# tum-pbs/differentiable-piso

Hardware: AMD Instinct MI355X
Metric: PISO steps/s (fwd+adjoint) at 2048^2 staggered grid (higher is better)
Workload: dtype f64

## Files before the change

### differentiable-piso_amd/csrc/cg.hip

```cpp
#include <atomic>
#include "cg_kernels.h"
#include "cg_driver.h"
#include "cg_tiny.h"
#include "options.h"
#include <cstdio>
#include <vector>

namespace piso {

struct CgProfile {
  int enabled = 0, stride = 8;
  double ms[4] = {0, 0, 0, 0};
  long long count[4] = {0, 0, 0, 0};
};
static CgProfile g_prof;

struct HostPoll {
  CgState* pinned = nullptr;
  hipEvent_t ev[2] = {nullptr, nullptr};
  hipEvent_t seg_ev[2] = {nullptr, nullptr};
  int cus = 0;
};
static std::atomic<unsigned> g_persist_launches{0};
static int g_persist_fallbacks = 0;
static thread_local int tl_xcd_map[kPersistMaxGrid];
static thread_local int tl_xcd_map_n = 0;
static long long g_tiny_solves = 0;
enum { DI_PATH = 0, DI_SIZEOF_T, DI_SIZEOF_CT, DI_V, DI_RECON, DI_SYMMETRIC, DI_ROWS_PER_WAVE, DI_K1_GRID, DI_K1_TILES, DI_R, DI_NQ,
       DI_WAVES, DI_LAUNCH_GRID, DI_PADDED, DI_XCD_LOCAL, DI_FELL_BACK, DI_TINY_PER_X, DI_K2_GRID, DI_SEGMENTS, DI_COUNT };
static thread_local int tl_dispatch[DI_COUNT];
static thread_local int tl_dispatch_n = 0;
static bool g_xcd_local_failed = false;
static long long g_verify_runs = 0;
static int g_verify_failures = 0;
constexpr int kPollDevices = 16;
static thread_local HostPoll tl_poll_dev[kPollDevices];
static thread_local HostPoll* tl_poll_cur = &tl_poll_dev[0];
#define tl_poll (*tl_poll_cur)

static int ensure_poll() {
  int dev = 0;
  PISO_HIP_CHECK(hipGetDevice(&dev));
  if (dev < 0 || dev >= kPollDevices) { set_error_msg("piso_cg_solve: device ordinal out of range"); return PISO_ERR_INVALID_ARG; }
  tl_poll_cur = &tl_poll_dev[dev];
  if (!tl_poll.pinned) {
    PISO_HIP_CHECK(hipHostMalloc(reinterpret_cast<void**>(&tl_poll.pinned), 2 * sizeof(CgState), hipHostMallocDefault));
    PISO_HIP_CHECK(hipEventCreateWithFlags(&tl_poll.ev[0], hipEventDisableTiming));
    PISO_HIP_CHECK(hipEventCreateWithFlags(&tl_poll.ev[1], hipEventDisableTiming));
    PISO_HIP_CHECK(hipDeviceGetAttribute(&tl_poll.cus, hipDeviceAttributeMultiprocessorCount, dev));
  }
  return PISO_OK;
}

constexpr size_t kPadMaxCells = (size_t)1 << 19;
static bool padded_dims(int nx, int ny, int per_x, int per_y, int elem, int* nxp, int* nyp) {
  *nxp = nx; *nyp = ny;
  if (elem != 8 || nx % 2 != 0 || nx < 8 || ny < 8) return false;
  const bool pad_x = nx % 128 != 0, pad_y = ny % 2 != 0;
  if (!pad_x && !pad_y) return false;
  const int px = (nx + 127) / 128 * 128;
  int py = (ny + 3) / 4 * 4;
  if (px != nx && per_x) return false;
  if (py != ny && per_y) {
    py = ny;
    if (ny % 2 != 0 || ((long long)(px / 128) * (ny / 2)) % 2 != 0) return false;
  }
  if ((size_t)px * py > kPadMaxCells) return false;
  *nxp = px; *nyp = py;
  return true;
}

template <typename T>
struct CgCarve { T *cC, *oT; float* oF; int* flags; T *b_pad, *x_pad; unsigned* persist_ws; };
template <typename T>
static CgCarve<T> cg_carve(Arena& ar, size_t n, bool padded, CgArgs<T>& a) {
  CgCarve<T> c;
  c.cC = ar.take<T>(n);
  c.oT = ar.take<T>(4 * n);
  c.oF = ar.take<float>(4 * n);
  c.flags = ar.take<int>(4);
  c.b_pad = padded ? ar.take<T>(n) : nullptr;
  c.x_pad = padded ? ar.take<T>(n) : nullptr;
  a.r = ar.take<T>(n); a.z = ar.take<T>(n); a.p[0] = ar.take<T>(n); a.p[1] = ar.take<T>(n);
  a.zp[0] = ar.take<T>(n); a.zp[1] = ar.take<T>(n);
  a.partsA = ar.take<T>(3 * kMaxPartials); a.partsB = ar.take<T>(3 * kMaxPartials); a.partsS = ar.take<T>(kMaxPartials);
  a.scal = ar.take<T>(SC_COUNT);
  a.state = ar.take<CgState>(2);
  c.persist_ws = ar.take<unsigned>(kPersistWsWordsAll);
  return c;
}

template <typename T>
static size_t cg_workspace_bytes(int nx_in, int ny_in) {
  int nx = nx_in, ny = ny_in;
  const bool padded = padded_dims(nx_in, ny_in, 0, 0, (int)sizeof(T), &nx, &ny);
  Arena ar = counting_arena();
  CgArgs<T> a;
  cg_carve<T>(ar, (padded ? 3 : 1) * (size_t)nx * ny, false, a);
  return counted_bytes(ar);
}

static void record_dispatch(int path, size_t state_bytes, size_t coef_bytes, int tiny_per_x, int V = 0, bool recon = false, bool symmetric = false,
                            const CgTiling* t = nullptr, const PersistPlan* p = nullptr, bool fell_back = false) {
  int* d = tl_dispatch;
  for (int i = 0; i < DI_COUNT; ++i) d[i] = 0;
  d[DI_PATH] = path; d[DI_SIZEOF_T] = (int)state_bytes; d[DI_SIZEOF_CT] = (int)coef_bytes; d[DI_TINY_PER_X] = tiny_per_x;
  d[DI_V] = V; d[DI_RECON] = recon ? 1 : 0; d[DI_SYMMETRIC] = symmetric ? 1 : 0; d[DI_FELL_BACK] = fell_back ? 1 : 0;
  if (t) { d[DI_ROWS_PER_WAVE] = t->rows_per_wave; d[DI_K1_GRID] = t->g1; d[DI_K1_TILES] = t->k1_tiles; d[DI_K2_GRID] = t->g2; }
  if (p) d[DI_PADDED] = p->ragged ? 1 : 0;
  if (p && p->R) { d[DI_R] = p->R; d[DI_NQ] = p->NQ; d[DI_WAVES] = p->waves; d[DI_LAUNCH_GRID] = p->launch_grid; d[DI_XCD_LOCAL] = p->xcd_local ? 1 : 0; }
  tl_dispatch_n = DI_COUNT;
}

struct EventPool {
  static constexpr int kMax = 64;
  hipEvent_t start[2][kMax], stop[2][kMax];
  int used[2] = {0, 0};
  bool created = false;
};
static thread_local EventPool tl_events;
struct SegmentTimes { double ms = 0; long long iters = 0, launches = 0; };

static int ensure_events(EventPool& ep) {
  if (ep.created) return PISO_OK;
  for (int q = 0; q < 2; ++q)
    for (int i = 0; i < EventPool::kMax; ++i) {
      PISO_HIP_CHECK(hipEventCreate(&ep.start[q][i]));
      PISO_HIP_CHECK(hipEventCreate(&ep.stop[q][i]));
    }
  ep.created = true;
  return PISO_OK;
}

static int read_profile(const EventPool& ep, const SegmentTimes& seg, float* kernel_ms_out) {
  double ms[2] = {0, 0};
  for (int q = 0; q < 2; ++q)
    for (int i = 0; i < ep.used[q]; ++i) {
      float t = 0;
      PISO_HIP_CHECK(hipEventElapsedTime(&t, ep.start[q][i], ep.stop[q][i]));
      ms[q] += t;
    }
  if (kernel_ms_out) {
    kernel_ms_out[0] = ep.used[0] ? (float)(ms[0] / ep.used[0]) : 0.f;
    kernel_ms_out[1] = ep.used[1] ? (float)(ms[1] / ep.used[1]) : 0.f;
  }
  if (g_prof.enabled) {
    for (int q = 0; q < 2; ++q) { g_prof.ms[q] += ms[q]; g_prof.count[q] += ep.used[q]; }
    g_prof.ms[2] += seg.ms; g_prof.count[2] += seg.iters; g_prof.count[3] += seg.launches;
  }
  if (kernel_ms_out && seg.iters > 0) { kernel_ms_out[0] = (float)(seg.ms / seg.iters); kernel_ms_out[1] = 0.f; }
  return PISO_OK;
}

struct PersistTiming {
  unsigned long long* ticks = nullptr;
  ~PersistTiming() { if (ticks) (void)hipFree(ticks); }
};
static int print_persist_timing(const unsigned long long* ticks, int grid, int k_last) {
  std::vector<unsigned long long> h(12 * grid);
  PISO_HIP_CHECK(hipMemcpy(h.data(), ticks, h.size() * sizeof(unsigned long long), hipMemcpyDeviceToHost));
  const char* names[9] = {"D (p update, stencil, sums, publish)", "exchange", "U (stencil, x / r update, ring)", "-", "-",
                           "  exchange: wave sums + drain of the perimeter stores", "  exchange: first barrier", "  exchange: publish + polling",
                           "  exchange: record sums + second barrier"};
  const double f = 0.01 / (double)(k_last > 0 ? k_last : 1);
  if (opt(OPT_CG_PERSIST_TIMING) >= 2) {
    for (int b = 0; b < grid; ++b)
      fprintf(stderr, "cg_persist_wg %3d xcd %d band %3d  D %.2f  exchange %.2f  U %.2f  | drain %.2f  barrier1 %.2f  publish+poll %.2f  sums %.2f\n", b, (int)h[9 * grid + b], (int)h[10 * grid + b],
              f * (double)h[0 * grid + b], f * (double)h[1 * grid + b], f * (double)h[2 * grid + b],
              f * (double)h[5 * grid + b], f * (double)h[6 * grid + b], f * (double)h[7 * grid + b], f * (double)h[8 * grid + b]);
  }
  for (int q = 0; q < 9; ++q) {
    double s = 0, mn = 1e300, mx = 0;
    for (int b = 0; b < grid; ++b) { const double v = (double)h[q * grid + b]; s += v; mn = v < mn ? v : mn; mx = v > mx ? v : mx; }
    fprintf(stderr, "cg_persist %s: avg %.2f us/iter  min %.2f  max %.2f\n", names[q], f * s / grid, f * mn, f * mx);
  }
  return PISO_OK;
}

template <typename T, typename CT>
static int verify_residual(const CgArgs<T>& a, const PersistCtl& pc, hipStream_t stream, bool* failed) {
  unsigned* out2 = reinterpret_cast<unsigned*>(pc.err) + 4;
  PISO_HIP_CHECK(hipMemsetAsync(out2, 0, 2 * sizeof(unsigned), stream));
  const int gvf = grid_for((long long)a.nx * a.ny, kBlock * 4, 1024);
  cg_verify_sum_x<T><<<gvf, kBlock, 0, stream>>>(a, a.partsA);
  cg_verify_gap<T, CT><<<gvf, kBlock, 0, stream>>>(a, a.partsA, gvf, out2);
  PISO_LAUNCH_CHECK();
  unsigned h2[2] = {0, 0};
  PISO_HIP_CHECK(hipMemcpyAsync(h2, out2, sizeof(h2), hipMemcpyDeviceToHost, stream));
  PISO_HIP_CHECK(hipStreamSynchronize(stream));
  float gap, scale;
  memcpy(&gap, &h2[0], 4); memcpy(&scale, &h2[1], 4);
  ++g_verify_runs;
  *failed = (gap > 1e-5f * scale && gap > 1e-30f) || opt(OPT_CG_VERIFY) == 2;
  return PISO_OK;
}

static int inspect_poll(int slot, int* stop_it) {
  hipError_t e = hipEventSynchronize(tl_poll.ev[slot]);
  if (e != hipSuccess) { set_error("hipEventSynchronize", e); return -1; }
  if (tl_poll.pinned[slot].done) { *stop_it = tl_poll.pinned[slot].iterations; return 1; }
  return 0;
}
static int poll_batch(size_t n) {
  const double t_iter_us = (double)n * 120.0 / 4.0e6;
  const int batch = (int)(1000.0 / (t_iter_us < 8.0 ? 8.0 : t_iter_us));
  return batch < 10 ? 10 : (batch > 200 ? 200 : batch);
}

template <typename T, typename CT, int V, bool RECON>
struct GpuLink {
  CgArgs<T> a;
  hipStream_t stream;
  bool fixed, prof;
  CgTiling tile;
  PersistPlan plan;
  PersistCtl pc;
  PersistTiming timing;
  int seg_len, batch, prof_stride, polls = 0, unsynced = 0;
  bool sample = false;
  SegmentTimes seg;
  EventPool& ep = tl_events;

  int start(unsigned* persist_ws, bool symmetric, int rank_deficient, bool allow_persist) {
    const size_t n = (size_t)a.nx * a.ny;
    tile = cg_tile(a, V, opt(OPT_CG_RPW), opt(OPT_CG_MAXBLOCKS));
    PISO_TRY(ensure_poll());
    if (prof) PISO_TRY(ensure_events(ep));
    ep.used[0] = ep.used[1] = 0;
    prof_stride = g_prof.stride > 0 ? g_prof.stride : 8;
    cg_init<T><<<tile.gflat, kBlock, 0, stream>>>(a, rank_deficient);
    PISO_LAUNCH_CHECK();
    batch = poll_batch(n);
    plan = persist_plan(PersistQuery{a.nx, a.ny, V, a.per_y, a.nx_true != 0, sizeof(T), sizeof(CT), RECON, symmetric, false, tl_poll.cus,
                                     opt(OPT_CG_PERSIST), opt(OPT_CG_PERSIST_R), opt(OPT_CG_PERSIST_HALF), opt(OPT_CG_PERSIST_NQ),
                                     opt(OPT_CG_XCD_LOCAL), g_xcd_local_failed, allow_persist});
    PISO_TRY((persist_prepare<T, CT, RECON, false>(plan, tl_poll.cus, pc, persist_ws, stream)));
    if (plan.R && kPersistDiag && opt_on(OPT_CG_PERSIST_TIMING)) {
      PISO_HIP_CHECK(hipMalloc(reinterpret_cast<void**>(&timing.ticks), 12 * plan.launch_grid * sizeof(unsigned long long)));
      PISO_HIP_CHECK(hipMemsetAsync(timing.ticks, 0, 12 * plan.launch_grid * sizeof(unsigned long long), stream));
      pc.timing = timing.ticks;
    }
    record_dispatch(plan.R ? 3 : 2, sizeof(T), sizeof(CT), 0, V, RECON, symmetric, &tile, &plan, !allow_persist);
    seg_len = persist_segment_len(n, opt(OPT_CG_SEGMENT));
    hipEvent_t* seg_ev = tl_poll.seg_ev;
    if (plan.R && prof && !seg_ev[0]) { PISO_HIP_CHECK(hipEventCreate(&seg_ev[0])); PISO_HIP_CHECK(hipEventCreate(&seg_ev[1])); }
    return PISO_OK;
  }

  bool persistent() const { return plan.R != 0; }
  int segment(int k, int ke, CgLoop& st) {
    hipEvent_t* seg_ev = tl_poll.seg_ev;
    if (prof) PISO_HIP_CHECK(hipEventRecord(seg_ev[0], stream));
    PISO_TRY((persist_launch<T, CT, RECON, false>(plan, a, pc, g_persist_launches.fetch_add(1, std::memory_order_relaxed), k, ke, st.sv, st.pending, NoSlab{}, stream)));
    if (prof) PISO_HIP_CHECK(hipEventRecord(seg_ev[1], stream));
    const bool defer = !prof && ke - k <= 32 && unsynced + (ke - k) <= 256 && ke < st.total;
    unsynced = defer ? unsynced + (ke - k) : 0;
    if (defer) return PISO_OK;
    PISO_HIP_CHECK(hipMemcpyAsync(&tl_poll.pinned[0], &a.state[0], sizeof(CgState), hipMemcpyDeviceToHost, stream));
    int herr = 0;
    PISO_HIP_CHECK(hipMemcpyAsync(&herr, pc.err, sizeof(int), hipMemcpyDeviceToHost, stream));
    PISO_HIP_CHECK(hipStreamSynchronize(stream));
    if (herr) {
      ++g_persist_fallbacks;
      if (plan.xcd_local) g_xcd_local_failed = true;
      return kPersistRetry;
    }
    const CgState& hst = tl_poll.pinned[0];
    if (prof) {
      const int ran = hst.done ? (hst.iterations - k > 0 ? hst.iterations - k : 0) : ke - k;
      float t = 0; PISO_HIP_CHECK(hipEventElapsedTime(&t, seg_ev[0], seg_ev[1])); seg.ms += t; seg.iters += ran < ke - k ? ran : ke - k; ++seg.launches;
    }
    if (hst.done) { st.finished = true; st.stop_it = hst.iterations; }
    return PISO_OK;
  }

  int k1(int k, int mode, int sv, int chk, int pend) {
    sample = prof && mode == MODE_NORMAL && (k % prof_stride == prof_stride - 1) && ep.used[0] < EventPool::kMax;
    if (sample) PISO_HIP_CHECK(hipEventRecord(ep.start[0][ep.used[0]], stream));
    cg_k1<T, CT, V, RECON><<<tile.g1, kBlock, 0, stream>>>(a, k, mode, sv, chk, pend);
    if (sample) PISO_HIP_CHECK(hipEventRecord(ep.stop[0][ep.used[0]++], stream));
    return PISO_OK;
  }
  int k2(int k, int sv) {
    if (sample) PISO_HIP_CHECK(hipEventRecord(ep.start[1][ep.used[1]], stream));
    cg_k2<T, V><<<tile.g2, kBlock, 0, stream>>>(a, k, sv);
    if (sample) PISO_HIP_CHECK(hipEventRecord(ep.stop[1][ep.used[1]++], stream));
    return PISO_OK;
  }
  int flush(int k, int sv) { cg_flush_x<T><<<tile.gflat, kBlock, 0, stream>>>(a, k, sv); return PISO_OK; }
  int reset_residual(int sv) { cg_reset_residual<T><<<tile.gflat, kBlock, 0, stream>>>(a, sv); return PISO_OK; }
  int halo(int) { return PISO_OK; }

  int poll(CgLoop& st, bool now) {
    const int slot = polls & 1;
    PISO_HIP_CHECK(hipMemcpyAsync(&tl_poll.pinned[slot], &a.state[st.sv & 1], sizeof(CgState), hipMemcpyDeviceToHost, stream));
    PISO_HIP_CHECK(hipEventRecord(tl_poll.ev[slot], stream));
    if (now || polls > 0) {
      const int r = inspect_poll(now ? slot : (polls - 1) & 1, &st.stop_it);
      if (r < 0) return PISO_ERR_HIP;
      if (r > 0) st.finished = true;
    }
    ++polls;
    return PISO_OK;
  }
  int look(int k, CgLoop& st) { return (!fixed && (k + 1) % batch == 0 && k + 1 < st.total) ? poll(st, false) : PISO_OK; }

  int finish(CgLoop& st) {
    if (!fixed && !st.finished) PISO_TRY(poll(st, true));
    PISO_HIP_CHECK(hipStreamSynchronize(stream));
    if (opt(OPT_CG_XCD_MAP) == 1) {
      tl_xcd_map_n = 0;
      if (st.segments_run > 0 && !plan.xcd_local && plan.grid <= kPersistMaxGrid) {
        PISO_HIP_CHECK(hipMemcpy(tl_xcd_map, pc.xcd + kPersistXcdTable, (size_t)plan.grid * sizeof(int), hipMemcpyDeviceToHost));
        tl_xcd_map_n = plan.grid;
      }
    }
    if (st.segments_run > 0) {
      int herr = 0;
      PISO_HIP_CHECK(hipMemcpy(&herr, pc.err, sizeof(int), hipMemcpyDeviceToHost));
      if (herr) { ++g_persist_fallbacks; return kPersistRetry; }
    }
    if (st.segments_run > 0 && sizeof(T) == 8 && !fixed && opt(OPT_CG_VERIFY) != 0) {
      bool failed = false;
      PISO_TRY((verify_residual<T, CT>(a, pc, stream, &failed)));
      if (failed) { ++g_verify_failures; ++g_persist_fallbacks; return kPersistRetry; }
    }
    if (timing.ticks) PISO_TRY(print_persist_timing(timing.ticks, plan.grid, st.k_last));
    tl_dispatch[DI_SEGMENTS] = st.segments_run;
    return PISO_OK;
  }
};

template <typename T>
__global__ __launch_bounds__(kBlock) void cg_copy_rows(const T* __restrict__ src, T* __restrict__ dst, int nx, int ny, int ld_src, int ld_dst) {
  const size_t n = (size_t)nx * ny;
  for (size_t i = (size_t)blockIdx.x * kBlock + threadIdx.x; i < n; i += (size_t)gridDim.x * kBlock) {
    const size_t j = i / (size_t)nx, c = i % (size_t)nx;
    dst[j * (size_t)ld_dst + c] = src[j * (size_t)ld_src + c];
  }
}

template <typename T>
static int cg_solve(int nx, int ny, int per_x, int per_y, const T* L, const T* b, T* x_out, float accuracy,
                    int max_iterations, int rank_deficient, int reset, int fixed, int* iterations_out,
                    float* kernel_ms_out, void* ws, size_t ws_bytes, piso_stream_t stream_, int* iterations_dev = nullptr) {
  tl_dispatch_n = 0;
  if (nx < 1 || ny < 1 || !L || !b || !x_out || !ws || max_iterations < 0 || reset < 1) {
    set_error_msg("piso_cg_solve: invalid argument");
    return PISO_ERR_INVALID_ARG;
  }
  if (ws_bytes < cg_workspace_bytes<T>(nx, ny)) {
    set_error_msg("piso_cg_solve: workspace too small");
    return PISO_ERR_INVALID_ARG;
  }
  hipStream_t stream = static_cast<hipStream_t>(stream_);
  const size_t n_true = (size_t)nx * ny;
  if (n_true <= (size_t)kTinyMaxCells && opt(OPT_CG_TINY) != 0 && opt(OPT_CG_PERSIST) < 0) {
    CgState* st_dev = reinterpret_cast<CgState*>(ws);
    const int total = fixed ? fixed : max_iterations;
    hipEvent_t* ev = nullptr;
    if (kernel_ms_out) {
      { const int rc = ensure_poll(); if (rc != PISO_OK) return rc; }
      ev = tl_poll.seg_ev;
      if (!ev[0]) { PISO_HIP_CHECK(hipEventCreate(&ev[0])); PISO_HIP_CHECK(hipEventCreate(&ev[1])); }
      PISO_HIP_CHECK(hipEventRecord(ev[0], stream));
    }
    const bool async = iterations_dev != nullptr;
    const bool cols = nx <= 64 && ny <= kColsMaxNy && (!per_x || nx == 64) && opt(OPT_CG_TINY) != 2;
    if (cols && per_x)
      cg_tiny_cols<T, true><<<1, kTinyThreads, 0, stream>>>(L, b, x_out, nx, ny, per_y, fixed ? -1.0f : accuracy, total, fixed ? 0 : reset,
                                                            rank_deficient, st_dev, iterations_dev);
    else if (cols)
      cg_tiny_cols<T, false><<<1, kTinyThreads, 0, stream>>>(L, b, x_out, nx, ny, per_y, fixed ? -1.0f : accuracy, total, fixed ? 0 : reset,
                                                             rank_deficient, st_dev, iterations_dev);
    else
      cg_tiny<T><<<1, kTinyThreads, 0, stream>>>(L, b, x_out, nx, ny, per_x, per_y, fixed ? -1.0f : accuracy, total, fixed ? 0 : reset,
                                                 rank_deficient, st_dev, iterations_dev);
    PISO_LAUNCH_CHECK();
    ++g_tiny_solves;
    record_dispatch(cols ? 1 : 0, sizeof(T), sizeof(T), (cols && per_x) ? 1 : 0);
    if (async) return PISO_OK;
    if (ev) PISO_HIP_CHECK(hipEventRecord(ev[1], stream));
    CgState hst;
    PISO_HIP_CHECK(hipMemcpyAsync(&hst, st_dev, sizeof(CgState), hipMemcpyDeviceToHost, stream));
    PISO_HIP_CHECK(hipStreamSynchronize(stream));
    if (iterations_out) *iterations_out = (!fixed && hst.done) ? hst.iterations : total;
    if (ev) { float ms = 0; PISO_HIP_CHECK(hipEventElapsedTime(&ms, ev[0], ev[1])); kernel_ms_out[0] = total > 0 ? ms / (float)total : 0.f; kernel_ms_out[1] = 0.f; }
    return PISO_OK;
  }
  if (iterations_dev) {
    set_error_msg("piso_cg_solve_async: this grid is solved with the host in the loop (segments, stopping test): call piso_cg_solve");
    return PISO_ERR_NEEDS_HOST;
  }
  int nxp = nx, nyp = ny;
  const bool padded = opt(OPT_CG_PERSIST) != 0 && opt(OPT_CG_PAD) != 0 &&
                      padded_dims(nx, ny, per_x, per_y, (int)sizeof(T), &nxp, &nyp);
  const size_t n = (size_t)nxp * nyp;
  Arena ar(ws, ws_bytes);
  CgArgs<T> a;
  const CgCarve<T> c = cg_carve<T>(ar, n, padded, a);
  a.cC = c.cC;
  a.b = padded ? c.b_pad : b; a.x = padded ? c.x_pad : x_out;
  a.nx = nxp; a.ny = nyp; a.per_x = per_x; a.per_y = per_y;
  a.nx_true = padded ? nx : 0; a.ny_true = padded ? ny : 0; a.ncells = padded ? (double)n_true : 0.0;
  a.ntx = a.nty = a.rows_per_wave = 0; a.nA = a.nB = 0;
  a.accuracy = fixed ? -1.0f : accuracy;
  a.gA = nullptr; a.gB = nullptr;
  a.nt = 0;
  if (opt(OPT_CG_NT) > 0) a.nt = opt(OPT_CG_NT);
  if (!ar.ok()) { set_error_msg("piso_cg_solve: workspace too small"); return PISO_ERR_INVALID_ARG; }

  PISO_HIP_CHECK(hipMemsetAsync(c.flags, 0, 4 * sizeof(int), stream));
  cg_zero_partials<T><<<(3 * kMaxPartials + 255) / 256, 256, 0, stream>>>(a.partsA, a.partsB, a.partsS);
  const int gs = grid_for((long long)n_true, kBlock * 4);
  if (padded) {
    PISO_HIP_CHECK(hipMemsetAsync(c.cC, 0, n * sizeof(T), stream));
    PISO_HIP_CHECK(hipMemsetAsync(c.oT, 0, 4 * n * sizeof(T), stream));
    PISO_HIP_CHECK(hipMemsetAsync(c.oF, 0, 4 * n * sizeof(float), stream));
    PISO_HIP_CHECK(hipMemsetAsync(c.b_pad, 0, n * sizeof(T), stream));
    cg_copy_rows<T><<<gs, kBlock, 0, stream>>>(b, c.b_pad, nx, ny, nx, nxp);
  }
  cg_setup_coeffs<T><<<gs, kBlock, 0, stream>>>(L, c.cC, c.oT, c.oF, a.partsS, c.flags, n_true, nx, ny, per_x, per_y, padded ? nxp : 0, padded ? n : 0);
  PISO_LAUNCH_CHECK();
  int hflags[3] = {1, 1, 1};
  PISO_HIP_CHECK(hipMemcpyAsync(hflags, c.flags, 3 * sizeof(int), hipMemcpyDeviceToHost, stream));
  PISO_HIP_CHECK(hipStreamSynchronize(stream));
  const CgCoefs coefs = cg_coefs(hflags[0], hflags[1], hflags[2], opt_on(OPT_CG_NO_COMPACT), opt_on(OPT_CG_NO_RECON), opt_on(OPT_CG_NO_SYM));
  if (coefs.compact) { a.oS = c.oF; a.oW = c.oF + n; a.oE = c.oF + 2 * n; a.oN = c.oF + 3 * n; }
  else { a.oS = c.oT; a.oW = c.oT + n; a.oE = c.oT + 2 * n; a.oN = c.oT + 3 * n; }
  const bool aligned = ((reinterpret_cast<uintptr_t>(a.b) | reinterpret_cast<uintptr_t>(a.x)) & 15) == 0;
  const bool vec = aligned && (nxp % (16 / (int)sizeof(T)) == 0);
  const bool prof = (kernel_ms_out != nullptr) || g_prof.enabled;
  const int rc = cg_retry_without_segments("piso_cg_solve", [&](bool allow_persist) {
    return cg_with_instance<T>(coefs, vec, [&](auto inst) {
      using I = decltype(inst);
      GpuLink<T, typename I::CT, I::V, I::RECON> link{a, stream, fixed != 0, prof};
      PISO_TRY(link.start(c.persist_ws, coefs.symmetric, rank_deficient, allow_persist));
      PISO_TRY(cg_iterate(link, fixed ? fixed : max_iterations, reset, fixed != 0, iterations_out));
      return prof ? read_profile(link.ep, link.seg, kernel_ms_out) : PISO_OK;
    });
  });
  if (rc != PISO_OK) return rc;
  if (padded) {
    cg_copy_rows<T><<<gs, kBlock, 0, stream>>>(c.x_pad, x_out, nx, ny, nxp, nx);
    PISO_LAUNCH_CHECK();
    PISO_HIP_CHECK(hipStreamSynchronize(stream));
  }
  return PISO_OK;
}

}

using namespace piso;

extern "C" {

size_t piso_cg_workspace_bytes(int nx, int ny, int elem_size) {
  return elem_size == 8 ? cg_workspace_bytes<double>(nx, ny) : cg_workspace_bytes<float>(nx, ny);
}

int piso_cg_solve_f64(int nx, int ny, int periodic_x, int periodic_y, const double* laplace, const double* divergence,
                      double* x_out, float accuracy, int max_iterations, int rank_deficient, int residual_reset,
                      int* iterations_out, void* workspace, size_t workspace_bytes, piso_stream_t stream) {
  const piso::OptScope knobs;
  return cg_solve<double>(nx, ny, periodic_x, periodic_y, laplace, divergence, x_out, accuracy, max_iterations,
                          rank_deficient, residual_reset, 0, iterations_out, nullptr, workspace, workspace_bytes, stream);
}

int piso_cg_solve_f32(int nx, int ny, int periodic_x, int periodic_y, const float* laplace, const float* divergence,
                      float* x_out, float accuracy, int max_iterations, int rank_deficient, int residual_reset,
                      int* iterations_out, void* workspace, size_t workspace_bytes, piso_stream_t stream) {
  const piso::OptScope knobs;
  return cg_solve<float>(nx, ny, periodic_x, periodic_y, laplace, divergence, x_out, accuracy, max_iterations,
                         rank_deficient, residual_reset, 0, iterations_out, nullptr, workspace, workspace_bytes, stream);
}

int piso_cg_solve_async_f64(int nx, int ny, int periodic_x, int periodic_y, const double* laplace, const double* divergence,
                            double* x_out, float accuracy, int max_iterations, int rank_deficient, int residual_reset,
                            int* iterations_dev, void* workspace, size_t workspace_bytes, piso_stream_t stream) {
  const piso::OptScope knobs;
  if (!iterations_dev) { set_error_msg("piso_cg_solve_async: iterations_dev is NULL"); return PISO_ERR_INVALID_ARG; }
  return cg_solve<double>(nx, ny, periodic_x, periodic_y, laplace, divergence, x_out, accuracy, max_iterations,
                          rank_deficient, residual_reset, 0, nullptr, nullptr, workspace, workspace_bytes, stream, iterations_dev);
}

int piso_cg_solve_async_f32(int nx, int ny, int periodic_x, int periodic_y, const float* laplace, const float* divergence,
                            float* x_out, float accuracy, int max_iterations, int rank_deficient, int residual_reset,
                            int* iterations_dev, void* workspace, size_t workspace_bytes, piso_stream_t stream) {
  const piso::OptScope knobs;
  if (!iterations_dev) { set_error_msg("piso_cg_solve_async: iterations_dev is NULL"); return PISO_ERR_INVALID_ARG; }
  return cg_solve<float>(nx, ny, periodic_x, periodic_y, laplace, divergence, x_out, accuracy, max_iterations,
                         rank_deficient, residual_reset, 0, nullptr, nullptr, workspace, workspace_bytes, stream, iterations_dev);
}

int piso_cg_fixed_iterations_f64(int nx, int ny, int periodic_x, int periodic_y, const double* laplace,
                                 const double* divergence, double* x_out, int rank_deficient, int iterations,
                                 float* kernel_ms_out, void* workspace, size_t workspace_bytes, piso_stream_t stream) {
  const piso::OptScope knobs;
  if (iterations < 1) { set_error_msg("piso_cg_fixed_iterations: iterations < 1"); return PISO_ERR_INVALID_ARG; }
  return cg_solve<double>(nx, ny, periodic_x, periodic_y, laplace, divergence, x_out, 0.f, iterations, rank_deficient,
                          1 << 30, iterations, nullptr, kernel_ms_out, workspace, workspace_bytes, stream);
}

void piso_cg_profile_enable(int enable, int stride) {
  g_prof.enabled = enable;
  if (stride > 0) g_prof.stride = stride;
  for (int q = 0; q < 4; ++q) { g_prof.ms[q] = 0; g_prof.count[q] = 0; }
}

int piso_cg_persist_fallbacks(void) { return g_persist_fallbacks; }
int piso_cg_last_xcd_map(int* out, int capacity) {
  const int n = tl_xcd_map_n < capacity ? tl_xcd_map_n : capacity;
  for (int i = 0; i < n; ++i) out[i] = tl_xcd_map[i];
  return tl_xcd_map_n;
}
long long piso_cg_tiny_solves(void) { return g_tiny_solves; }
int piso_cg_last_dispatch(int* out, int capacity) {
  const int n = tl_dispatch_n < capacity ? tl_dispatch_n : capacity;
  for (int i = 0; i < n; ++i) out[i] = tl_dispatch[i];
  return tl_dispatch_n;
}
void piso_cg_verify_stats(long long* runs_out, int* failures_out) {
  if (runs_out) *runs_out = g_verify_runs;
  if (failures_out) *failures_out = g_verify_failures;
}

void piso_cg_profile_read(double* ms_sum, long long* count) {
  for (int q = 0; q < 4; ++q) { ms_sum[q] = g_prof.ms[q]; count[q] = g_prof.count[q]; }
}

}
```

### differentiable-piso_amd/csrc/cg_driver.h

```cpp
#pragma once
#include "cg_dispatch.h"

namespace piso {

enum CgStepKind { CG_SEGMENT, CG_RESET, CG_FIRST, CG_NORMAL };
struct CgStep { CgStepKind kind; int ke; };
inline CgStep cg_next_step(int k, int total, int reset, bool fixed, int seg_len, bool persistent) {
  const bool is_reset = !fixed && ((k + 1) % reset == 0);
  if (persistent && k > 0 && !is_reset) {
    int ke = total;
    if (!fixed) { const int next_reset = ((k + 1 + reset - 1) / reset) * reset - 1; if (next_reset < ke) ke = next_reset; }
    if (ke > k + seg_len) ke = k + seg_len;
    if (ke > k) return {CG_SEGMENT, ke};
  }
  return {is_reset ? CG_RESET : (k == 0 ? CG_FIRST : CG_NORMAL), k + 1};
}

struct CgCoefs { bool compact, recon, symmetric; };
inline CgCoefs cg_coefs(double not_f32, double not_recon, double not_sym, bool no_compact, bool no_recon, bool no_sym) {
  CgCoefs c;
  c.compact = not_f32 == 0 && !no_compact;
  c.recon = c.compact && not_recon == 0 && !no_recon;
  c.symmetric = not_sym == 0 && !no_sym;
  return c;
}

template <typename CT_, int V_, bool RECON_>
struct CgInstance { using CT = CT_; static constexpr int V = V_; static constexpr bool RECON = RECON_; };
template <typename T, typename F>
inline int cg_with_instance(const CgCoefs& c, bool vec, F&& f) {
  constexpr int VMID = 16 / sizeof(T);
  if (c.compact && c.recon) return vec ? f(CgInstance<float, VMID, true>{}) : f(CgInstance<float, 1, true>{});
  if (c.compact) return vec ? f(CgInstance<float, VMID, false>{}) : f(CgInstance<float, 1, false>{});
  return vec ? f(CgInstance<T, VMID, false>{}) : f(CgInstance<T, 1, false>{});
}

template <typename F>
inline int cg_retry_without_segments(const char* who, F&& attempt) {
  for (int i = 0; i < 2; ++i) {
    const int rc = attempt(i == 0);
    if (rc != kPersistRetry) return rc;
  }
  char msg[96];
  snprintf(msg, sizeof(msg), "%s: persistent segment failed twice", who);
  set_error_msg(msg);
  return PISO_ERR_HIP;
}

constexpr size_t kCgWsSlack = 40 * 1024;
inline Arena counting_arena() { return Arena(nullptr, ~(size_t)0); }
inline size_t counted_bytes(const Arena& ar) { return align_up(ar.used, 256) + kCgWsSlack; }

enum { HALO_R = 0, HALO_X = 1 };
struct CgLoop {
  int total;
  int sv = 0, k_last = -1, stop_it = -1, segments_run = 0;
  bool pending = false;
  bool finished = false;
};

template <typename Link>
inline int cg_iterate(Link& link, int total, int reset, bool fixed, int* iterations_out) {
  CgLoop st;
  st.total = total;
  for (int k = 0; k < total && !st.finished;) {
    const CgStep step = cg_next_step(k, total, reset, fixed, link.seg_len, link.persistent());
    if (step.kind == CG_SEGMENT) {
      PISO_TRY(link.segment(k, step.ke, st));
      ++st.segments_run;
      st.k_last = step.ke - 1;
      st.pending = false;
      k = step.ke;
      continue;
    }
    if (step.kind == CG_RESET) {
      if (st.pending) { PISO_TRY(link.flush(k - 1, st.sv)); st.pending = false; }
      PISO_TRY(link.halo(HALO_X));
      PISO_TRY(link.k1(k, MODE_RESET, st.sv, k > 0 ? 1 : 0, 0));
      ++st.sv;
      PISO_TRY(link.reset_residual(st.sv));
      PISO_TRY(link.halo(HALO_R));
      PISO_TRY(link.k1(k, MODE_INIT, st.sv, 0, 0));
    } else if (step.kind == CG_FIRST) {
      PISO_TRY(link.k1(k, MODE_INIT, st.sv, 0, 0));
    } else {
      PISO_TRY(link.k1(k, MODE_NORMAL, st.sv, 1, st.pending ? 1 : 0));
      ++st.sv;
    }
    PISO_TRY(link.k2(k, st.sv));
    PISO_TRY(link.halo(HALO_R));
    PISO_LAUNCH_CHECK();
    st.pending = true;
    st.k_last = k;
    PISO_TRY(link.look(k, st));
    ++k;
  }
  if (st.pending && st.k_last >= 0) PISO_TRY(link.flush(st.k_last, st.sv));
  PISO_TRY(link.finish(st));
  if (iterations_out) *iterations_out = st.finished ? st.stop_it : total;
  return PISO_OK;
}

}
```

### differentiable-piso_amd/csrc/options.h

```cpp
#pragma once

namespace piso {

enum Opt {
  OPT_CG_PERSIST = 0,
  OPT_CG_PERSIST_R,
  OPT_CG_PERSIST_HALF,
  OPT_CG_PERSIST_NQ,
  OPT_CG_SEGMENT,
  OPT_CG_PERSIST_TIMING,
  OPT_CG_RPW,
  OPT_CG_MAXBLOCKS,
  OPT_CG_NT,
  OPT_CG_NO_COMPACT,
  OPT_CG_NO_RECON,
  OPT_CG_NO_SYM,
  OPT_CG_VERIFY,
  OPT_CG_PAD,
  OPT_CG_XCD_LOCAL,
  OPT_CG_TINY,
  OPT_CG_XCD_MAP,
  OPT_CONV_LDS,
  OPT_BICG_FOLD,
  OPT_BICG_SWEEP_LDS,
  OPT_BICG_FUSE_P,
  OPT_SLAB_FORCE,
  OPT_SLAB_HOP_TICKS,
  OPT_MG_TAIL,
  OPT_MG_CHECK_EVERY,
  OPT_MG_SLAB_GATHER_CELLS,
  OPT_MG_F32_VEC,
  OPT_COUNT
};

int opt(Opt o);
inline bool opt_on(Opt o) { return opt(o) > 0; }

struct OptScope {
  OptScope();
  ~OptScope();
  OptScope(const OptScope&) = delete;
  OptScope& operator=(const OptScope&) = delete;
};

}
```

### differentiable-piso_amd/csrc/runtime.hip

```cpp
#include "piso_common.h"
#include "options.h"
#include <stdlib.h>
#include <atomic>

namespace piso {
static thread_local char g_err[512] = "";
void set_error(const char* what, hipError_t err) {
  snprintf(g_err, sizeof(g_err), "%s: %s", what, hipGetErrorString(err));
}
void set_error_msg(const char* what) { snprintf(g_err, sizeof(g_err), "%s", what); }

static const char* const kOptNames[OPT_COUNT] = {"cg_persist", "cg_persist_r", "cg_persist_half", "cg_persist_nq", "cg_segment", "cg_persist_timing",
                                                 "cg_rpw", "cg_maxblocks", "cg_nt", "cg_no_compact", "cg_no_recon", "cg_no_sym", "cg_verify", "cg_pad", "cg_xcd_local", "cg_tiny", "cg_xcd_map", "conv_lds", "bicg_fold", "bicg_sweep_lds", "bicg_fuse_p", "slab_force", "slab_hop_ticks", "mg_tail", "mg_check_every", "mg_slab_gather_cells", "mg_f32_vec"};
struct Options {
  std::atomic<int> v[OPT_COUNT];
  Options() {
    for (int i = 0; i < OPT_COUNT; ++i) {
      char env[64] = "PISO_";
      size_t k = 5;
      for (const char* c = kOptNames[i]; *c && k + 1 < sizeof(env); ++c) env[k++] = (char)((*c >= 'a' && *c <= 'z') ? *c - 32 : *c);
      env[k] = 0;
      const char* e = getenv(env);
      v[i].store((e && *e) ? atoi(e) : -1, std::memory_order_relaxed);
    }
    if (getenv("PISO_CG_NO_PERSIST")) v[OPT_CG_PERSIST].store(0, std::memory_order_relaxed);
  }
};
static Options g_opt;
static thread_local int tl_snapshot[OPT_COUNT];
static thread_local int tl_scope_depth = 0;
int opt(Opt o) { return tl_scope_depth > 0 ? tl_snapshot[o] : g_opt.v[o].load(std::memory_order_relaxed); }
OptScope::OptScope() {
  if (tl_scope_depth++ == 0)
    for (int i = 0; i < OPT_COUNT; ++i) tl_snapshot[i] = g_opt.v[i].load(std::memory_order_relaxed);
}
OptScope::~OptScope() { --tl_scope_depth; }
static int opt_index(const char* name) {
  if (!name) return -1;
  for (int i = 0; i < OPT_COUNT; ++i)
    if (strcmp(name, kOptNames[i]) == 0) return i;
  return -1;
}
}

extern "C" {
const char* piso_version(void) { return "libpiso_hip 0.1 (gfx950)"; }
const char* piso_last_error_string(void) { return piso::g_err; }
int piso_set_option(const char* name, int value) {
  const int i = piso::opt_index(name);
  if (i < 0) { piso::set_error_msg("piso_set_option: unknown option"); return PISO_ERR_INVALID_ARG; }
  piso::g_opt.v[i].store(value, std::memory_order_relaxed);
  return PISO_OK;
}
int piso_get_option(const char* name, int* value_out) {
  const int i = piso::opt_index(name);
  if (i < 0 || !value_out) { piso::set_error_msg("piso_get_option: unknown option"); return PISO_ERR_INVALID_ARG; }
  *value_out = piso::g_opt.v[i].load(std::memory_order_relaxed);
  return PISO_OK;
}
int piso_device_count(void) {
  int n = 0;
  if (hipGetDeviceCount(&n) != hipSuccess) return 0;
  return n;
}
}
```

Before: 5.339.

## Defer persistent CG convergence checks one segment behind to overlap host syncs

Each persistent CG segment now queues its state and error copies into pinned double-buffered slots with an event, instead of synchronizing the stream right after the launch. The host reads the previous segment's result only after launching the next one, so the GPU keeps running while the host waits. The end-of-solve state read, error read and residual verification are also batched into a single stream synchronize. In exchange, one extra segment may be queued after convergence; it is counted as idle, and a new option can turn the look-behind off.

```diff
diff --git a/differentiable-piso_amd/csrc/cg.hip b/differentiable-piso_amd/csrc/cg.hip
--- a/differentiable-piso_amd/csrc/cg.hip
+++ b/differentiable-piso_amd/csrc/cg.hip
@@ -15,12 +15,16 @@
 };
 static CgProfile g_prof;
 
+struct SegLook { CgState st; int err; unsigned gap[2]; };
 struct HostPoll {
   CgState* pinned = nullptr;
+  SegLook* looks = nullptr;
   hipEvent_t ev[2] = {nullptr, nullptr};
-  hipEvent_t seg_ev[2] = {nullptr, nullptr};
+  hipEvent_t look_ev[2] = {nullptr, nullptr};
+  hipEvent_t seg_ev[4] = {nullptr, nullptr, nullptr, nullptr};
   int cus = 0;
 };
+constexpr int kSegLooks = 3;
 static std::atomic<unsigned> g_persist_launches{0};
 static int g_persist_fallbacks = 0;
 static thread_local int tl_xcd_map[kPersistMaxGrid];
@@ -44,9 +48,13 @@
   if (dev < 0 || dev >= kPollDevices) { set_error_msg("piso_cg_solve: device ordinal out of range"); return PISO_ERR_INVALID_ARG; }
   tl_poll_cur = &tl_poll_dev[dev];
   if (!tl_poll.pinned) {
-    PISO_HIP_CHECK(hipHostMalloc(reinterpret_cast<void**>(&tl_poll.pinned), 2 * sizeof(CgState), hipHostMallocDefault));
-    PISO_HIP_CHECK(hipEventCreateWithFlags(&tl_poll.ev[0], hipEventDisableTiming));
-    PISO_HIP_CHECK(hipEventCreateWithFlags(&tl_poll.ev[1], hipEventDisableTiming));
+    static_assert(sizeof(CgState) % alignof(SegLook) == 0, "SegLook records follow the two CgState records");
+    PISO_HIP_CHECK(hipHostMalloc(reinterpret_cast<void**>(&tl_poll.pinned), 2 * sizeof(CgState) + kSegLooks * sizeof(SegLook), hipHostMallocDefault));
+    tl_poll.looks = reinterpret_cast<SegLook*>(tl_poll.pinned + 2);
+    for (int i = 0; i < 2; ++i) {
+      PISO_HIP_CHECK(hipEventCreateWithFlags(&tl_poll.ev[i], hipEventDisableTiming));
+      PISO_HIP_CHECK(hipEventCreateWithFlags(&tl_poll.look_ev[i], hipEventDisableTiming));
+    }
     PISO_HIP_CHECK(hipDeviceGetAttribute(&tl_poll.cus, hipDeviceAttributeMultiprocessorCount, dev));
   }
   return PISO_OK;
@@ -178,21 +186,21 @@
 }
 
 template <typename T, typename CT>
-static int verify_residual(const CgArgs<T>& a, const PersistCtl& pc, hipStream_t stream, bool* failed) {
+static int queue_verify_residual(const CgArgs<T>& a, const PersistCtl& pc, hipStream_t stream, unsigned* h2) {
   unsigned* out2 = reinterpret_cast<unsigned*>(pc.err) + 4;
   PISO_HIP_CHECK(hipMemsetAsync(out2, 0, 2 * sizeof(unsigned), stream));
   const int gvf = grid_for((long long)a.nx * a.ny, kBlock * 4, 1024);
   cg_verify_sum_x<T><<<gvf, kBlock, 0, stream>>>(a, a.partsA);
   cg_verify_gap<T, CT><<<gvf, kBlock, 0, stream>>>(a, a.partsA, gvf, out2);
   PISO_LAUNCH_CHECK();
-  unsigned h2[2] = {0, 0};
-  PISO_HIP_CHECK(hipMemcpyAsync(h2, out2, sizeof(h2), hipMemcpyDeviceToHost, stream));
-  PISO_HIP_CHECK(hipStreamSynchronize(stream));
+  PISO_HIP_CHECK(hipMemcpyAsync(h2, out2, 2 * sizeof(unsigned), hipMemcpyDeviceToHost, stream));
+  return PISO_OK;
+}
+static bool verify_residual_failed(const unsigned* h2) {
   float gap, scale;
   memcpy(&gap, &h2[0], 4); memcpy(&scale, &h2[1], 4);
   ++g_verify_runs;
-  *failed = (gap > 1e-5f * scale && gap > 1e-30f) || opt(OPT_CG_VERIFY) == 2;
-  return PISO_OK;
+  return (gap > 1e-5f * scale && gap > 1e-30f) || opt(OPT_CG_VERIFY) == 2;
 }
 
 static int inspect_poll(int slot, int* stop_it) {
@@ -217,6 +225,8 @@
   PersistCtl pc;
   PersistTiming timing;
   int seg_len, batch, prof_stride, polls = 0, unsynced = 0;
+  int looks = 0, idle_segments = 0, look_k[2] = {0, 0}, look_ke[2] = {0, 0};
+  bool in_flight = false;
   bool sample = false;
   SegmentTimes seg;
   EventPool& ep = tl_events;
@@ -243,34 +253,64 @@
     record_dispatch(plan.R ? 3 : 2, sizeof(T), sizeof(CT), 0, V, RECON, symmetric, &tile, &plan, !allow_persist);
     seg_len = persist_segment_len(n, opt(OPT_CG_SEGMENT));
     hipEvent_t* seg_ev = tl_poll.seg_ev;
-    if (plan.R && prof && !seg_ev[0]) { PISO_HIP_CHECK(hipEventCreate(&seg_ev[0])); PISO_HIP_CHECK(hipEventCreate(&seg_ev[1])); }
+    if (plan.R && prof)
+      for (int i = 0; i < 4; ++i)
+        if (!seg_ev[i]) PISO_HIP_CHECK(hipEventCreate(&seg_ev[i]));
     return PISO_OK;
   }
 
   bool persistent() const { return plan.R != 0; }
+  int queue_look(int slot, int k, int ke) {
+    SegLook* h = &tl_poll.looks[slot];
+    PISO_HIP_CHECK(hipMemcpyAsync(&h->st, &a.state[0], sizeof(CgState), hipMemcpyDeviceToHost, stream));
+    PISO_HIP_CHECK(hipMemcpyAsync(&h->err, pc.err, sizeof(int), hipMemcpyDeviceToHost, stream));
+    PISO_HIP_CHECK(hipEventRecord(tl_poll.look_ev[slot], stream));
+    look_k[slot] = k; look_ke[slot] = ke;
+    return PISO_OK;
+  }
+  int read_look(int slot, CgLoop& st) {
+    const SegLook& h = tl_poll.looks[slot];
+    const int k = look_k[slot], ke = look_ke[slot];
+    if (h.err) {
+      ++g_persist_fallbacks;
+      if (plan.xcd_local) g_xcd_local_failed = true;
+      return kPersistRetry;
+    }
+    if (st.finished) { ++idle_segments; return PISO_OK; }
+    if (prof) {
+      const int ran = h.st.done ? (h.st.iterations - k > 0 ? h.st.iterations - k : 0) : ke - k;
+      float t = 0; PISO_HIP_CHECK(hipEventElapsedTime(&t, tl_poll.seg_ev[2 * slot], tl_poll.seg_ev[2 * slot + 1]));
+      seg.ms += t; seg.iters += ran < ke - k ? ran : ke - k; ++seg.launches;
+    }
+    if (h.st.done) { st.finished = true; st.stop_it = h.st.iterations; }
+    return PISO_OK;
+  }
   int segment(int k, int ke, CgLoop& st) {
-    hipEvent_t* seg_ev = tl_poll.seg_ev;
+    if (cg_look_before_launch(in_flight, st.pending)) {
+      PISO_HIP_CHECK(hipEventSynchronize(tl_poll.look_ev[(looks - 1) & 1]));
+      in_flight = false;
+      PISO_TRY(read_look((looks - 1) & 1, st));
+      if (st.finished) { ++idle_segments; return PISO_OK; }
+    }
+    const int slot = looks & 1;
+    hipEvent_t* seg_ev = tl_poll.seg_ev + 2 * slot;
     if (prof) PISO_HIP_CHECK(hipEventRecord(seg_ev[0], stream));
     PISO_TRY((persist_launch<T, CT, RECON, false>(plan, a, pc, g_persist_launches.fetch_add(1, std::memory_order_relaxed), k, ke, st.sv, st.pending, NoSlab{}, stream)));
     if (prof) PISO_HIP_CHECK(hipEventRecord(seg_ev[1], stream));
-    const bool defer = !prof && ke - k <= 32 && unsynced + (ke - k) <= 256 && ke < st.total;
-    unsynced = defer ? unsynced + (ke - k) : 0;
-    if (defer) return PISO_OK;
-    PISO_HIP_CHECK(hipMemcpyAsync(&tl_poll.pinned[0], &a.state[0], sizeof(CgState), hipMemcpyDeviceToHost, stream));
-    int herr = 0;
-    PISO_HIP_CHECK(hipMemcpyAsync(&herr, pc.err, sizeof(int), hipMemcpyDeviceToHost, stream));
-    PISO_HIP_CHECK(hipStreamSynchronize(stream));
-    if (herr) {
-      ++g_persist_fallbacks;
-      if (plan.xcd_local) g_xcd_local_failed = true;
-      return kPersistRetry;
-    }
-    const CgState& hst = tl_poll.pinned[0];
-    if (prof) {
-      const int ran = hst.done ? (hst.iterations - k > 0 ? hst.iterations - k : 0) : ke - k;
-      float t = 0; PISO_HIP_CHECK(hipEventElapsedTime(&t, seg_ev[0], seg_ev[1])); seg.ms += t; seg.iters += ran < ke - k ? ran : ke - k; ++seg.launches;
-    }
-    if (hst.done) { st.finished = true; st.stop_it = hst.iterations; }
+    const CgSegLook lk = cg_segment_look(k, ke, st.total, unsynced, prof, opt(OPT_CG_LOOK_BEHIND) != 0);
+    unsynced = lk.copy ? 0 : unsynced + (ke - k);
+    const int before = in_flight ? (looks - 1) & 1 : -1;
+    if (lk.copy) { PISO_TRY(queue_look(slot, k, ke)); ++looks; in_flight = true; }
+    if (before >= 0) {
+      PISO_HIP_CHECK(hipEventSynchronize(tl_poll.look_ev[before]));
+      if (!lk.copy) in_flight = false;
+      PISO_TRY(read_look(before, st));
+    }
+    if (lk.copy && lk.wait) {
+      PISO_HIP_CHECK(hipStreamSynchronize(stream));
+      in_flight = false;
+      PISO_TRY(read_look(slot, st));
+    }
     return PISO_OK;
   }
 
@@ -306,8 +346,18 @@
   int look(int k, CgLoop& st) { return (!fixed && (k + 1) % batch == 0 && k + 1 < st.total) ? poll(st, false) : PISO_OK; }
 
   int finish(CgLoop& st) {
-    if (!fixed && !st.finished) PISO_TRY(poll(st, true));
+    SegLook* end = &tl_poll.looks[kSegLooks - 1];
+    const bool want_state = !fixed && !st.finished;
+    const bool want_verify = st.segments_run > 0 && sizeof(T) == 8 && !fixed && opt(OPT_CG_VERIFY) != 0;
+    end->err = 0;
+    if (want_state) PISO_HIP_CHECK(hipMemcpyAsync(&end->st, &a.state[st.sv & 1], sizeof(CgState), hipMemcpyDeviceToHost, stream));
+    if (st.segments_run > 0) PISO_HIP_CHECK(hipMemcpyAsync(&end->err, pc.err, sizeof(int), hipMemcpyDeviceToHost, stream));
+    if (want_verify) PISO_TRY((queue_verify_residual<T, CT>(a, pc, stream, end->gap)));
     PISO_HIP_CHECK(hipStreamSynchronize(stream));
+    if (in_flight) { in_flight = false; PISO_TRY(read_look((looks - 1) & 1, st)); }
+    if (end->err) { ++g_persist_fallbacks; return kPersistRetry; }
+    if (want_state && !st.finished && end->st.done) { st.finished = true; st.stop_it = end->st.iterations; }
+    if (want_verify && verify_residual_failed(end->gap)) { ++g_verify_failures; ++g_persist_fallbacks; return kPersistRetry; }
     if (opt(OPT_CG_XCD_MAP) == 1) {
       tl_xcd_map_n = 0;
       if (st.segments_run > 0 && !plan.xcd_local && plan.grid <= kPersistMaxGrid) {
@@ -315,18 +365,8 @@
         tl_xcd_map_n = plan.grid;
       }
     }
-    if (st.segments_run > 0) {
-      int herr = 0;
-      PISO_HIP_CHECK(hipMemcpy(&herr, pc.err, sizeof(int), hipMemcpyDeviceToHost));
-      if (herr) { ++g_persist_fallbacks; return kPersistRetry; }
-    }
-    if (st.segments_run > 0 && sizeof(T) == 8 && !fixed && opt(OPT_CG_VERIFY) != 0) {
-      bool failed = false;
-      PISO_TRY((verify_residual<T, CT>(a, pc, stream, &failed)));
-      if (failed) { ++g_verify_failures; ++g_persist_fallbacks; return kPersistRetry; }
-    }
     if (timing.ticks) PISO_TRY(print_persist_timing(timing.ticks, plan.grid, st.k_last));
-    tl_dispatch[DI_SEGMENTS] = st.segments_run;
+    tl_dispatch[DI_SEGMENTS] = st.segments_run - idle_segments;
     return PISO_OK;
   }
 };
diff --git a/differentiable-piso_amd/csrc/cg_driver.h b/differentiable-piso_amd/csrc/cg_driver.h
--- a/differentiable-piso_amd/csrc/cg_driver.h
+++ b/differentiable-piso_amd/csrc/cg_driver.h
@@ -1,5 +1,6 @@
 #pragma once
 #include "cg_dispatch.h"
+#include "cg_segment_look.h"
 
 namespace piso {
 
diff --git a/differentiable-piso_amd/csrc/cg_segment_look.h b/differentiable-piso_amd/csrc/cg_segment_look.h
--- /dev/null
+++ b/differentiable-piso_amd/csrc/cg_segment_look.h
@@ -0,0 +1,13 @@
+#pragma once
+
+namespace piso {
+
+struct CgSegLook { bool copy, wait; };
+inline CgSegLook cg_segment_look(int k, int ke, int total, int unsynced, bool prof, bool look_behind) {
+  const bool defer = !prof && ke - k <= 32 && unsynced + (ke - k) <= 256 && ke < total;
+  return {!defer, !defer && !look_behind};
+}
+
+inline bool cg_look_before_launch(bool in_flight, bool pending) { return in_flight && pending; }
+
+}
diff --git a/differentiable-piso_amd/csrc/options.h b/differentiable-piso_amd/csrc/options.h
--- a/differentiable-piso_amd/csrc/options.h
+++ b/differentiable-piso_amd/csrc/options.h
@@ -30,6 +30,7 @@
   OPT_MG_CHECK_EVERY,
   OPT_MG_SLAB_GATHER_CELLS,
   OPT_MG_F32_VEC,
+  OPT_CG_LOOK_BEHIND,
   OPT_COUNT
 };
 
diff --git a/differentiable-piso_amd/csrc/runtime.hip b/differentiable-piso_amd/csrc/runtime.hip
--- a/differentiable-piso_amd/csrc/runtime.hip
+++ b/differentiable-piso_amd/csrc/runtime.hip
@@ -11,7 +11,7 @@
 void set_error_msg(const char* what) { snprintf(g_err, sizeof(g_err), "%s", what); }
 
 static const char* const kOptNames[OPT_COUNT] = {"cg_persist", "cg_persist_r", "cg_persist_half", "cg_persist_nq", "cg_segment", "cg_persist_timing",
-                                                 "cg_rpw", "cg_maxblocks", "cg_nt", "cg_no_compact", "cg_no_recon", "cg_no_sym", "cg_verify", "cg_pad", "cg_xcd_local", "cg_tiny", "cg_xcd_map", "conv_lds", "bicg_fold", "bicg_sweep_lds", "bicg_fuse_p", "slab_force", "slab_hop_ticks", "mg_tail", "mg_check_every", "mg_slab_gather_cells", "mg_f32_vec"};
+                                                 "cg_rpw", "cg_maxblocks", "cg_nt", "cg_no_compact", "cg_no_recon", "cg_no_sym", "cg_verify", "cg_pad", "cg_xcd_local", "cg_tiny", "cg_xcd_map", "conv_lds", "bicg_fold", "bicg_sweep_lds", "bicg_fuse_p", "slab_force", "slab_hop_ticks", "mg_tail", "mg_check_every", "mg_slab_gather_cells", "mg_f32_vec", "cg_look_behind"};
 struct Options {
   std::atomic<int> v[OPT_COUNT];
   Options() {
```

Result: no change. 5.320 (-0.4%).
